# Medical-Image-Analysis-Laboratory/fetalsyngen

Measured on AMD Instinct MI355X. Metric: synthetic volumes/sec at 256^3 (full deform+GMM+blur+resample path), higher is better.
Workload: dtype f32; 1 GPU; BASELINE configs[1]: single 256^3 label volume per step, full path, all gates on; rng=keyed, outputs=fp32 [0,1] image + fp32 labels in HBM, volumes_per_rank=936, parallelism=1 independent replicas (no collective), streams_per_gpu=1

## Files before the change

### fetalsyngen_amd/_build.py

```python
from __future__ import annotations

import os
import shutil
import subprocess
from pathlib import Path

PKG = Path(__file__).resolve().parent
CSRC = PKG / "csrc"
LIB = PKG / "libfsg_hip.so"
SOURCES = ["fsg_deform.hip", "fsg_warp_lean.hip", "fsg_zoom.hip", "fsg_intensity.hip", "fsg_blur.hip", "fsg_blur_rs.hip", "fsg_reduce.hip", "fsg_slice_acq.hip", "fsg_slice_acq_bwd.hip", "fsg_slice_acq_adjoint_bwd.hip", "fsg_artifacts.hip", "fsg_keyed.hip", "fsg_codes.hip", "fsg_seedgen.hip",
           "fsg_regrid.hip", "fsg_pick.hip", "fsg_pipeline.cpp"]
EXTRA = os.environ.get("FSG_EXTRA_FLAGS", "").split()
FLAGS = ["-O3", "--offload-arch=gfx950", "-ffp-contract=off", "-fPIC", "-std=c++17", "-Wall", "-Wno-unused-function"]


def hipcc() -> str:
    exe = shutil.which("hipcc") or "/opt/rocm/bin/hipcc"
    if not os.path.exists(exe):
        raise RuntimeError("hipcc not found: libfsg_hip.so cannot be built")
    return exe


def needs_build() -> bool:
    if not LIB.exists():
        return True
    t = LIB.stat().st_mtime
    deps = [CSRC / s for s in SOURCES] + [CSRC / "fsg_common.h", CSRC / "fsg_sa.h", PKG.parent / "include" / "fsg_hip.h"]
    return any(d.stat().st_mtime > t for d in deps)


def build(force: bool = False, verbose: bool = False) -> Path:
    if not force and not needs_build():
        return LIB
    cc = hipcc()
    objs, jobs = [], []
    build_dir = PKG / "build"
    build_dir.mkdir(exist_ok=True)
    for s in SOURCES:
        o = build_dir / (s + ".o")
        lang = ["-x", "hip"] if s.endswith(".cpp") else []
        cmd = [cc, *FLAGS, *EXTRA, *lang, "-c", str(CSRC / s), "-o", str(o)]
        objs.append(str(o))
        deps = [CSRC / s, CSRC / "fsg_common.h", CSRC / "fsg_sa.h", PKG.parent / "include" / "fsg_hip.h", Path(__file__)]
        if not force and not EXTRA and o.exists() and all(d.stat().st_mtime < o.stat().st_mtime for d in deps):
            continue
        jobs.append(cmd)
    from concurrent.futures import ThreadPoolExecutor

    def run(cmd):
        if verbose:
            print(" ".join(cmd))
        subprocess.run(cmd, check=True)

    with ThreadPoolExecutor(max_workers=min(4, max(len(jobs), 1))) as pool:
        list(pool.map(run, jobs))
    tmp = LIB.with_suffix(".so.tmp")
    subprocess.run([cc, "-shared", "-fPIC", "--offload-arch=gfx950", *objs, "-o", str(tmp)], check=True)
    os.replace(tmp, LIB)
    return LIB


if __name__ == "__main__":
    print(build(force=True, verbose=True))
```

### fetalsyngen_amd/csrc/fsg_deform.hip

```cpp
#include "fsg_common.h"
#include "fsg_ride.h"

int g_tuning_flags = 0;

namespace {

__global__ __launch_bounds__(256) void coords_minmax_kernel(FsgDeformK D, int32_t* __restrict__ mm6) {
  float lo[3] = {INFINITY, INFINITY, INFINITY}, hi[3] = {-INFINITY, -INFINITY, -INFINITY};
  const int rows = D.n0 * D.n1;
  for (int r = blockIdx.x; r < rows; r += gridDim.x) {
    const int i = r / D.n1, j = r - i * D.n1;
    for (int k = threadIdx.x; k < D.n2; k += blockDim.x) {
      float x, y, z;
      fsg_position(D, i, j, k, x, y, z);
      lo[0] = fminf(lo[0], x); hi[0] = fmaxf(hi[0], x);
      lo[1] = fminf(lo[1], y); hi[1] = fmaxf(hi[1], y);
      lo[2] = fminf(lo[2], z); hi[2] = fmaxf(hi[2], z);
    }
  }
  __shared__ float red[6][4];
  const int wave = threadIdx.x >> 6, lane = threadIdx.x & 63;
#pragma unroll
  for (int a = 0; a < 3; ++a) {
    float l = fsg_wave_min(lo[a]), h = fsg_wave_max(hi[a]);
// ... 270 lines not shown
    float v = red[a][0];
    for (int w = 1; w < 4; ++w) v = fminf(v, red[a][w]);
    fsg_atomic_min_key(&mm3[a], v);
  }
}

__global__ __launch_bounds__(256) void coords_faces_min_kernel(FsgDeformK D, int32_t* __restrict__ mm3) {
  __shared__ float red[3][4];
  coords_faces_min_body(D, mm3, red, blockIdx.x, gridDim.x);
}

struct HeadGmm {
  const uint8_t* l0; const uint8_t* l1; const uint8_t* l2; const uint8_t* l3;
  size_t n;
  const float* mus; const float* sigmas; int ntab;
  const float* noise; uint64_t seed, stream_id;
  float* out;
  int ntuples, stride;
  uint32_t sel;
};

__global__ __launch_bounds__(256) __attribute__((amdgpu_waves_per_eu(8, 8))) void sample_head_kernel(HeadGmm G, FsgDeformK D, EpiK E, float* __restrict__ rows,
                                                          int stride, int rows_gx, int nrows, int nfaces,
                                                          int32_t* __restrict__ mm3) {
  __shared__ float s_mu[256], s_sg[256];
  __shared__ float red[3][4];
  union HeadSmem {
    RowsSmem rows;
    float2 code_ms[FSG_CODES_MAX];
  };
  __shared__ HeadSmem U;
  RowsSmem& S = U.rows;
  int b = blockIdx.x;
  if (b < nfaces) {
    coords_faces_min_body(D, mm3, red, b, nfaces);
    return;
  }
  b -= nfaces;
  if (b < nrows) {
    deform_rows_block(D, E, rows, stride, b / rows_gx, (b % rows_gx) * RB_J, S);
    return;
  }
  b -= nrows;
  if (G.ntuples > 0) {
    const fsg_ride::GmmCodesK C{G.l0, G.l1, G.ntuples, G.stride, G.sel, G.n, G.mus, G.sigmas, G.ntab, G.seed, G.stream_id, G.out};
    fsg_ride::gmm_codes_job(C, U.code_ms, (unsigned)b, gridDim.x - (unsigned)(nrows + nfaces));
    return;
  }
  for (int t = threadIdx.x; t < 256; t += blockDim.x) {
    s_mu[t] = t < G.ntab ? G.mus[t] : 0.f;
    s_sg[t] = t < G.ntab ? G.sigmas[t] : 0.f;
  }
  __syncthreads();
  fsg_gmm_x4_loop(G.l0, G.l1, G.l2, G.l3, G.n, s_mu, s_sg, G.noise, G.seed, G.stream_id, G.out, (unsigned)b,
                  gridDim.x - (unsigned)(nrows + nfaces));
}

constexpr int WARP_ROWS_PER_WAVE = 4;

#ifndef FSG_WARP_BATCH
#define FSG_WARP_BATCH 2
#endif
#ifndef FSG_WARP_NO_SKIP_OUTSIDE
#define FSG_WARP_SKIP_OUTSIDE 1
#endif

template <typename LT, bool HAS_LIN, bool HAS_NN, bool FAST, int Q0, int NQ>
__device__ __forceinline__ void warp_emitN(const FsgDeformK& D, const EpiK& E, const Margins& m, const float* sm,
                                           int nf, int i, int j, int kbase, const fsg_tap (&ck)[4],
                                           const fsg_tap (&cbk)[4], size_t row, const float* __restrict__ src_lin,
                                           float* __restrict__ out_lin, const LT* __restrict__ src_nn,
                                           LT* __restrict__ out_nn) {
  const float hx = (float)(D.n0 - 1), hy = (float)(D.n1 - 1), hz = (float)(D.n2 - 1);
  const unsigned sx = (unsigned)D.n1 * (unsigned)D.n2, sy = (unsigned)D.n2;
  float x[NQ], y[NQ], z[NQ];
#pragma unroll
  for (int q = 0; q < NQ; ++q) {
    const int k = min(kbase + 64 * (Q0 + q), D.n2 - 1);
// ... 240 lines not shown
    fsg_tap ck[4] = {none, none, none, none}, cbk[4] = {none, none, none, none};
#pragma unroll
    for (int q = 0; q < PATCH_NQ; ++q) {
      const int k = min(kk + 64 * q, D.n2 - 1);
      ck[q] = tap_at(s_tz, D.tz, D.field != nullptr, k);
      cbk[q] = tap_at(s_bz, E.bz, E.bias != nullptr, k);
    }
    if (live_row)
      warp_emitN<LT, HAS_LIN, HAS_NN, FAST, 0, PATCH_NQ>(D, E, m, sm, nf, i, j, kk, ck, cbk, row, src_lin, out_lin, src_nn,
                                                         out_nn);
    __syncthreads();
  }
}

template <bool MIN_ONLY>
__device__ __forceinline__ void coords_minmax_rows_body(const FsgDeformK& D, int32_t* __restrict__ mm6, int rows_per_block, int blk);

template <bool MIN_ONLY>
__global__ __launch_bounds__(256) void coords_minmax_rows_kernel(FsgDeformK D, int32_t* __restrict__ mm6,
                                                                 int rows_per_block) {
  coords_minmax_rows_body<MIN_ONLY>(D, mm6, rows_per_block, (int)blockIdx.x);
}

__global__ __launch_bounds__(256) void floormin_ride_kernel(FsgDeformK D, int32_t* __restrict__ mm6, int rows_per_block, int nrest,
                                                            const fsg_ride::DrawK P) {
  if ((int)blockIdx.x < nrest) coords_minmax_rows_body<true>(D, mm6, rows_per_block, (int)blockIdx.x);
  else fsg_ride::keyed_draw_body(P, (int)blockIdx.x - nrest);
}

template <bool MIN_ONLY>
__device__ __forceinline__ void coords_minmax_rows_body(const FsgDeformK& D, int32_t* __restrict__ mm6, int rows_per_block, int blk) {
  if (MIN_ONLY) {
    const int32_t one = fsg_f2key(1.0f);
    const int32_t k0 = __hip_atomic_load(&mm6[0], __ATOMIC_RELAXED, __HIP_MEMORY_SCOPE_AGENT);
    const int32_t k1 = __hip_atomic_load(&mm6[1], __ATOMIC_RELAXED, __HIP_MEMORY_SCOPE_AGENT);
    const int32_t k2 = __hip_atomic_load(&mm6[2], __ATOMIC_RELAXED, __HIP_MEMORY_SCOPE_AGENT);
    if (k0 < one && k1 < one && k2 < one) return;
  }
  __shared__ float sm_all[4][ROWCAP];
  __shared__ float red[6][4];
  const int wave = __builtin_amdgcn_readfirstlane(threadIdx.x >> 6), lane = threadIdx.x & 63;
  float* sm = sm_all[wave];
  float lo[3] = {INFINITY, INFINITY, INFINITY}, hi[3] = {-INFINITY, -INFINITY, -INFINITY};
  const int rows = D.n0 * D.n1;
  const int r_begin = blk * rows_per_block;
  const int r_end = min(rows, r_begin + rows_per_block);
  const fsg_tap none = fsg_tap{0, 0, 0.f, 0.f};
  const bool cached = D.n2 <= 256;
  fsg_tap ck[4];
  if (cached) {
#pragma unroll
    for (int q = 0; q < 4; ++q) {
// ... 239 lines not shown
    grid = (rows + rpb - 1) / rpb;
    hipLaunchKernelGGL(coords_minmax_rows_kernel<true>, dim3(grid), dim3(256), 0, st, D, mm3, rpb);
  } else {
    return FSG_E_TOOBIG;
  }
  FSG_RETURN_LAUNCH();
}

int fsg_coords_floormin_rest_f32(const fsg_deform* d, int32_t* mm3, void* stream) {
  FsgDeformK D;
  int rc = fsg_fill_deform(d, D);
  if (rc) return rc;
  if (!mm3) return FSG_E_BADARG;
  if ((D.field ? 3 * D.f2 : 0) > ROWCAP) return FSG_E_TOOBIG;
  const int rows = D.n0 * D.n1;
  int grid = (rows + 7) / 8 < 512 ? (rows + 7) / 8 : 512;
  const int rpb = (rows + grid - 1) / grid;
  grid = (rows + rpb - 1) / rpb;
  hipLaunchKernelGGL(coords_minmax_rows_kernel<true>, dim3(grid), dim3(256), 0, fsg_stream(stream), D, mm3, rpb);
  FSG_RETURN_LAUNCH();
}

static int launch_sample_head(const HeadGmm& G, size_t n, const fsg_deform* d, const fsg_epilogue* epi, float* rows,
                              int row_stride, int32_t* mm3, void* stream);

extern "C" int fsg_internal_floormin_rest_ride(const fsg_deform* d, int32_t* mm3, const void* drawk, unsigned draw_blocks, void* stream) {
  FsgDeformK D;
  int rc = fsg_fill_deform(d, D);
  if (rc) return rc;
  if (!mm3 || !drawk || draw_blocks == 0 || draw_blocks > 4096) return FSG_E_BADARG;
  if ((D.field ? 3 * D.f2 : 0) > ROWCAP) return FSG_E_TOOBIG;
  const int rows = D.n0 * D.n1;
  int grid = (rows + 7) / 8 < 512 ? (rows + 7) / 8 : 512;
  const int rpb = (rows + grid - 1) / grid;
  grid = (rows + rpb - 1) / rpb;
  hipLaunchKernelGGL(floormin_ride_kernel, dim3((unsigned)grid + draw_blocks), dim3(256), 0, fsg_stream(stream), D, mm3, rpb, grid,
                     *reinterpret_cast<const fsg_ride::DrawK*>(drawk));
  FSG_RETURN_LAUNCH();
}

extern "C" int fsg_internal_head_no_gmm(size_t n, const fsg_deform* d, const fsg_epilogue* epi, float* rows, int row_stride,
                                        int32_t* mm3, void* stream) {
  if (n == 0 || !mm3) return FSG_E_BADARG;
  HeadGmm G{};
  G.n = n;
  return launch_sample_head(G, n, d, epi, rows, row_stride, mm3, stream);
}

int fsg_sample_head_f32(const uint8_t* l0, const uint8_t* l1, const uint8_t* l2, const uint8_t* l3, size_t n,
                        const float* mus, const float* sigmas, int ntab, const float* noise, uint64_t seed,
                        uint64_t stream_id, float* out, const fsg_deform* d, const fsg_epilogue* epi, float* rows,
                        int row_stride, int32_t* mm3, void* stream) {
  if (n == 0 || !l0 || !mus || !sigmas || !out || ntab <= 0 || ntab > 256 || !mm3) return FSG_E_BADARG;
  const uintptr_t al = (uintptr_t)l0 | (uintptr_t)l1 | (uintptr_t)l2 | (uintptr_t)l3;
  if ((al & 3) || ((uintptr_t)out & 15)) return FSG_E_ALIGN;
  HeadGmm G{l0, l1, l2, l3, n, mus, sigmas, ntab, noise, seed, stream_id, out, 0, 0, 0u};
  return launch_sample_head(G, n, d, epi, rows, row_stride, mm3, stream);
}

int fsg_sample_head_codes_f32(const uint16_t* codes, const uint8_t* tuples, int ntuples, int stride, const int32_t sel[4],
                              size_t n, const float* mus, const float* sigmas, int ntab, uint64_t seed, uint64_t stream_id,
                              float* out, const fsg_deform* d, const fsg_epilogue* epi, float* rows, int row_stride,
                              int32_t* mm3, void* stream) {
  if (n == 0 || !codes || !tuples || !sel || !mus || !sigmas || !out || ntab <= 0 || ntab > 256 || !mm3) return FSG_E_BADARG;
  if (ntuples <= 0 || stride <= 0 || stride > 256) return FSG_E_BADARG;
  for (int m = 0; m < 4; ++m)
    if (sel[m] < 0 || sel[m] >= stride) return FSG_E_BADARG;
  if (ntuples > FSG_CODES_MAX || n > ((size_t)1 << 30)) return FSG_E_TOOBIG;
  if ((n & 7) || ((uintptr_t)codes & 15) || ((uintptr_t)out & 15)) return FSG_E_ALIGN;
  HeadGmm G{reinterpret_cast<const uint8_t*>(codes), tuples, nullptr, nullptr, n, mus, sigmas, ntab, nullptr, seed, stream_id, out,
            ntuples, stride, (uint32_t)sel[0] | ((uint32_t)sel[1] << 8) | ((uint32_t)sel[2] << 16) | ((uint32_t)sel[3] << 24)};
  return launch_sample_head(G, n, d, epi, rows, row_stride, mm3, stream);
}

static int launch_sample_head(const HeadGmm& G, size_t n, const fsg_deform* d, const fsg_epilogue* epi, float* rows,
                              int row_stride, int32_t* mm3, void* stream) {
  FsgDeformK D;
  int rc = fsg_fill_deform(d, D);
  if (rc) return rc;
  EpiK E;
  rc = fill_epilogue(epi, E);
  if (rc) return rc;
  const int need = (D.field ? 3 * D.f2 : 0) + (E.bias ? E.b2 : 0);
  if (need > 0 && (!rows || row_stride < need)) return FSG_E_BADARG;
  if ((size_t)D.n0 * D.n1 * D.n2 != n) return FSG_E_BADARG;
  if ((D.field ? 3 * D.f2 : 0) > ROWCAP) return FSG_E_TOOBIG;
  if (!rows_block_fits(D, E)) return FSG_E_TOOBIG;
  const int rows_gx = need > 0 ? (D.n1 + RB_J - 1) / RB_J : 0;
  const long long nrows = (long long)rows_gx * D.n0;
  const int faces = faces_total(D.n0, D.n1, D.n2);
  int nfaces = (faces + 255) / 256;
  if (nfaces > 1024) nfaces = 1024;
  size_t ngmm = ((n + 3) / 4 + 255) / 256;
  if (!G.out) ngmm = 0;
  if (ngmm > 4096) ngmm = 4096;
  if (nrows > 1000000) return FSG_E_TOOBIG;
  hipLaunchKernelGGL(sample_head_kernel, dim3((unsigned)(nrows + nfaces + ngmm)), dim3(256), 0, fsg_stream(stream), G, D,
                     E, rows, row_stride, rows_gx > 0 ? rows_gx : 1, (int)nrows, nfaces, mm3);
  FSG_RETURN_LAUNCH();
}

int fsg_coords_f32(const fsg_deform* d, const int32_t* mm6, float* xx, float* yy, float* zz, void* stream) {
  FsgDeformK D;
  int rc = fsg_fill_deform(d, D);
  if (rc) return rc;
  if (!mm6 || !xx || !yy || !zz) return FSG_E_BADARG;
  hipLaunchKernelGGL(coords_kernel, fsg_grid3(D.n0, D.n1, D.n2), fsg_block3(), 0, fsg_stream(stream), D, mm6, xx,
                     yy, zz);
  FSG_RETURN_LAUNCH();
}

int fsg_warp_f32(const fsg_deform* d, const int32_t* mm6, const float* src_lin, float* out_lin,
                 const float* src_nn, float* out_nn, const fsg_epilogue* epi, void* stream) {
  return launch_warp<float>(d, mm6, src_lin, out_lin, src_nn, out_nn, epi, stream);
}

int fsg_warp_f32_u8(const fsg_deform* d, const int32_t* mm6, const float* src_lin, float* out_lin,
                    const uint8_t* src_nn, uint8_t* out_nn, const fsg_epilogue* epi, void* stream) {
  return launch_warp<uint8_t>(d, mm6, src_lin, out_lin, src_nn, out_nn, epi, stream);
}

// ... 57 lines not shown
```

### fetalsyngen_amd/csrc/fsg_keyed.hip

```cpp
#include <hip/hip_runtime.h>
#include <cmath>
#include <cstring>
#include <new>
#include "fsg_common.h"
#include "fsg_ride.h"

namespace {

constexpr int KT_CAP = 1024;

struct KeyedCtx {
  fsg_keyed_config cfg;
  const fsg_tap* tab[4][3][KT_CAP + 1];
  int64_t block_bytes;
  int max_field[3], max_bias[3];
};

struct U4 { uint32_t x, y, z, w; };
inline U4 philox_host(uint32_t c0, uint32_t c1, uint32_t c2, uint32_t c3, uint32_t k0, uint32_t k1) {
  const uint32_t M0 = 0xD2511F53u, M1 = 0xCD9E8D57u, W0 = 0x9E3779B9u, W1 = 0xBB67AE85u;
  for (int r = 0; r < 10; ++r) {
    const uint64_t p0 = (uint64_t)M0 * c0, p1 = (uint64_t)M1 * c2;
    const uint32_t h0 = (uint32_t)(p0 >> 32), l0 = (uint32_t)p0, h1 = (uint32_t)(p1 >> 32), l1 = (uint32_t)p1;
    const uint32_t n0 = h1 ^ c1 ^ k0, n2 = h0 ^ c3 ^ k1;
// ... 161 lines not shown
  }
  if (slot_u(key, S_NOISE_GATE) < c.noise_prob || has(FSG_KO_NOISE_STD)) {
    d.noise_active = 1;
    d.noise_std = has(FSG_KO_NOISE_STD) ? o->noise_std : c.noise_std_min + (c.noise_std_max - c.noise_std_min) * slot_u(key, S_NOISE_STD);
    if (!std::isfinite(d.noise_std)) return FSG_E_BADARG;
    d.noise_std32 = (float)d.noise_std;
  }
  auto align256l = [](int64_t v) { return (v + 255) & ~(int64_t)255; };
  int64_t off = 0;
  d.off_mm8 = (int32_t)off; off = align256l(off + 8 * 4);
  d.off_slots = (int32_t)off; off = align256l(off + FSG_MM_NSLOTS * FSG_MM_SLOT_STRIDE * 4);
  d.off_mus = (int32_t)off; off = align256l(off + 256 * 4);
  d.off_sigmas = (int32_t)off; off = align256l(off + 256 * 4);
  d.off_bias = (int32_t)off; off = align256l(off + (d.bias_active ? (int64_t)d.bias_dims[0] * d.bias_dims[1] * d.bias_dims[2] * 4 : 0));
  if (off > 0x7FFFFF00LL) return FSG_E_TOOBIG;
  d.off_field = (int32_t)off; off = align256l(off + (d.nonlinear ? (int64_t)d.field_dims[0] * d.field_dims[1] * d.field_dims[2] * 12 : 0));
  if (off > 0x7FFFFF00LL) return FSG_E_TOOBIG;
  d.block_bytes = (int32_t)off;
  return 0;
}

using fsg_ride::DrawK;

__global__ __launch_bounds__(256) void keyed_draw_kernel(const DrawK P) { fsg_ride::keyed_draw_body(P, (int)blockIdx.x); }

int fill_draw(const KeyedCtx& C, const fsg_keyed_draws& d, void* block_dev, DrawK& P, unsigned& grid) {
  if (!block_dev || ((uintptr_t)block_dev & 15)) return FSG_E_BADARG;
  char* base = (char*)block_dev;
  P.key = d.key;
  P.mm8 = (int32_t*)(base + d.off_mm8);
  P.slots = (int32_t*)(base + d.off_slots);
  P.mus = (float*)(base + d.off_mus);
  P.sigmas = (float*)(base + d.off_sigmas);
  P.bias = (float*)(base + d.off_bias);
  P.field = (float*)(base + d.off_field);
  P.nlabels = C.cfg.nlabels; P.nseed = C.cfg.n_seed_labels; P.tie = C.cfg.tie_classes;
  P.nbias = d.bias_active ? d.bias_dims[0] * d.bias_dims[1] * d.bias_dims[2] : 0;
  P.nfield = d.nonlinear ? d.field_dims[0] * d.field_dims[1] * d.field_dims[2] * 3 : 0;
  P.bias_std = (float)d.bf_std;
  P.field_std = (float)d.nonlin_std;
  std::memcpy(P.seed_labels, C.cfg.seed_labels, 256);
  std::memcpy(P.gen_classes, C.cfg.generation_classes, 256);
  P.mus_in = (const float*)(uintptr_t)d.mus_in;
  P.sigmas_in = (const float*)(uintptr_t)d.sigmas_in;
  const int work = ((P.nbias + 3) >> 2) + ((P.nfield + 3) >> 2);
  grid = 1u + (unsigned)((work + 255) / 256);
  return 0;
}

int launch_draw(const KeyedCtx& C, const fsg_keyed_draws& d, void* block_dev, void* stream) {
  DrawK P;
  unsigned grid = 0;
  const int rc = fill_draw(C, d, block_dev, P, grid);
  if (rc) return rc;
  hipLaunchKernelGGL(keyed_draw_kernel, dim3(grid), dim3(256), 0, fsg_stream(stream), P);
  FSG_RETURN_LAUNCH();
}

}

extern "C" {

int fsg_keyed_create(const fsg_keyed_config* cfg, void** ctx) {
  if (!cfg || !ctx) return FSG_E_BADARG;
  const fsg_keyed_config& c = *cfg;
  for (int a = 0; a < 3; ++a)
    if (c.shape[a] <= 0 || c.shape[a] > KT_CAP || c.size[a] <= 0 || !(c.resolution[a] > 0)) return FSG_E_BADARG;
  if (c.meta_labels < 1 || c.meta_labels > 4 || c.min_subclusters < 1 || c.max_subclusters < c.min_subclusters ||
      c.max_subclusters - c.min_subclusters >= 16)
    return FSG_E_BADARG;
// ... 34 lines not shown
  KeyedCtx* K = (KeyedCtx*)ctx;
  if (!K || kind < 0 || kind > 3 || axis < 0 || axis > 2 || n < 1 || n > KT_CAP) return FSG_E_BADARG;
  K->tab[kind][axis][n] = table_dev;
  return 0;
}

int64_t fsg_keyed_block_bytes(void* ctx) { return ctx ? ((KeyedCtx*)ctx)->block_bytes : (int64_t)FSG_E_BADARG; }

int fsg_keyed_draw(void* ctx, uint64_t key, fsg_keyed_draws* out) {
  if (!ctx || !out) return FSG_E_BADARG;
  return draw(*(KeyedCtx*)ctx, key, nullptr, *out);
}

int fsg_keyed_draw_with(void* ctx, uint64_t key, const fsg_keyed_overrides* overrides, fsg_keyed_draws* out) {
  if (!ctx || !out) return FSG_E_BADARG;
  return draw(*(KeyedCtx*)ctx, key, overrides, *out);
}

int fsg_keyed_fill_block(void* ctx, const fsg_keyed_draws* d, void* block_dev, void* stream) {
  if (!ctx || !d) return FSG_E_BADARG;
  return launch_draw(*(KeyedCtx*)ctx, *d, block_dev, stream);
}

int fsg_keyed_sample_run(void* ctx, const int64_t* iv, int niv, fsg_keyed_draws* draws_out, void* stream) {
  KeyedCtx* K = (KeyedCtx*)ctx;
  if (!K || !iv || niv < FSG_KEYED_I_COUNT) return FSG_E_BADARG;
  const fsg_keyed_config& c = K->cfg;
  fsg_keyed_draws d;
  const bool ext = niv >= FSG_KEYED_I_COUNT_OV;
  const fsg_keyed_overrides* ov = ext ? (const fsg_keyed_overrides*)(uintptr_t)iv[FSG_KEYED_I_OVERRIDES] : nullptr;
  int rc = draw(*K, (uint64_t)iv[FSG_KEYED_I_KEY], ov, d);
  if (rc) return rc;
  if (draws_out) *draws_out = d;
  const int64_t cap = ext && iv[FSG_KEYED_I_BLOCK_BYTES] > 0 ? iv[FSG_KEYED_I_BLOCK_BYTES] : K->block_bytes;
  if (d.block_bytes > cap) return FSG_E_TOOBIG;
  char* base = (char*)(uintptr_t)iv[FSG_KEYED_I_BLOCK];
  if (!base) return FSG_E_BADARG;

  fsg_sample_plan q;
  std::memset(&q, 0, sizeof q);
  for (int a = 0; a < 3; ++a) q.shape[a] = c.shape[a];
  fsg_sample_image im;
  im.prior_in = (const float*)(uintptr_t)iv[FSG_KEYED_I_PRIOR_IN];
  im.image_in = (const float*)(uintptr_t)iv[FSG_KEYED_I_IMAGE_IN];
  im.image_out = (float*)(uintptr_t)iv[FSG_KEYED_I_IMAGE_OUT];
  if (im.image_in && !im.image_out) return FSG_E_BADARG;
// ... 84 lines not shown
  q.mm8_preset = 1;
  q.mm_slots = d.resample_active ? (int32_t*)(base + d.off_slots) : nullptr;
  q.mm_nslots = d.resample_active ? FSG_MM_NSLOTS : 0;
  q.out = (float*)(uintptr_t)iv[FSG_KEYED_I_OUT];
  q.trace_events = (void**)(uintptr_t)iv[FSG_KEYED_I_TRACE_EVENTS];
  q.trace_ids = (int32_t*)(uintptr_t)iv[FSG_KEYED_I_TRACE_IDS];
  q.trace_cap = (int32_t)iv[FSG_KEYED_I_TRACE_CAP];
  q.ev_blur_begin = (void*)(uintptr_t)iv[FSG_KEYED_I_EV_BLUR_BEGIN];
  q.ev_blur_end = (void*)(uintptr_t)iv[FSG_KEYED_I_EV_BLUR_END];

  const int64_t flags = iv[FSG_KEYED_I_FLAGS];
  const bool draw_done = (flags & 1) != 0 && !ov;
  DrawK next_draw;
  int32_t rode = 0;
  char* nbase = (char*)(uintptr_t)iv[FSG_KEYED_I_NEXT_BLOCK];
  if (nbase && (flags & 4)) {
    fsg_keyed_draws dn;
    rc = draw(*K, (uint64_t)iv[FSG_KEYED_I_NEXT_KEY], nullptr, dn);
    if (rc) return rc;
    if (dn.block_bytes > K->block_bytes) return FSG_E_TOOBIG;
    unsigned grid = 0;
    rc = fill_draw(*K, dn, nbase, next_draw, grid);
    if (rc) return rc;
    q.ride_draw = &next_draw;
    q.ride_draw_blocks = grid;
    q.rode = &rode;
  }

  if (!draw_done && q.trace_events && q.trace_ids && q.trace_cap > 1) {
    hipError_t e = hipEventRecord((hipEvent_t)q.trace_events[0], fsg_stream(stream));
    if (e != hipSuccess) return (int)e;
    q.trace_ids[0] = FSG_ST_BEGIN;
    q.trace_ids[q.trace_cap] = 1;
    q.trace_start = 1;
    q.trace_first_id = FSG_ST_DRAW;
  }
  if (!draw_done) {
    rc = launch_draw(*K, d, base, stream);
    if (rc) return rc;
  }
  rc = fsg_sample_run_image(&q, &im, stream);
  if (draws_out) draws_out->rode = rode;
  return rc;
}

}
```

### fetalsyngen_amd/csrc/fsg_pipeline.cpp

```cpp
#include <hip/hip_runtime.h>
#include <cstddef>
#include "../../include/fsg_hip.h"

extern "C" int fsg_internal_floormin_rest_ride(const fsg_deform* d, int32_t* mm3, const void* drawk, unsigned draw_blocks, void* stream);
extern "C" int fsg_internal_head_no_gmm(size_t n, const fsg_deform* d, const fsg_epilogue* epi, float* rows, int row_stride,
                                        int32_t* mm3, void* stream);


extern int g_tuning_flags;

extern "C" int fsg_pipeline_teardown(void) { return 0; }

#define FSG_TRY(expr)        \
  do {                       \
    int rc_ = (expr);        \
    if (rc_ != 0) return rc_; \
  } while (0)
#define FSG_HIP(expr)                          \
  do {                                         \
    hipError_t e_ = (expr);                    \
    if (e_ != hipSuccess) return (int)e_;      \
  } while (0)

extern "C" int fsg_sample_run(const fsg_sample_plan* p, void* stream) { return fsg_sample_run_image(p, nullptr, stream); }

extern "C" int fsg_sample_run_image(const fsg_sample_plan* p, const fsg_sample_image* im, void* stream) {
  if (!p || !p->out || !p->ws0 || !p->ws1 || !p->mm8) return FSG_E_BADARG;
  const int n0 = p->shape[0], n1 = p->shape[1], n2 = p->shape[2];
  if (n0 <= 0 || n1 <= 0 || n2 <= 0) return FSG_E_BADARG;
  const size_t n = (size_t)n0 * n1 * n2;
  if (n > (size_t)0x7FFFFFFF) return FSG_E_TOOBIG;
  const float* const image_in = im ? im->image_in : nullptr;
  float* const image_out = im ? im->image_out : nullptr;
  if (image_in && !image_out) return FSG_E_BADARG;
  const float* const prior = im ? im->prior_in : nullptr;
  hipStream_t st = (hipStream_t)stream;
  int rode = 0;
  if (p->rode) *p->rode = 0;

  int ntrace = p->trace_start > 0 ? p->trace_start : 0;
  auto mark = [&](int id) -> int {
    if (!p->trace_events || !p->trace_ids || ntrace >= p->trace_cap) return 0;
    hipError_t e = hipEventRecord((hipEvent_t)p->trace_events[ntrace], st);
    if (e != hipSuccess) return (int)e;
    p->trace_ids[ntrace++] = id;
    p->trace_ids[p->trace_cap] = ntrace;
    return 0;
  };
  FSG_TRY(mark(p->trace_start > 0 ? p->trace_first_id : FSG_ST_BEGIN));

  const bool has_gamma = p->epi.gamma > 0.f, has_bias = p->epi.bias != nullptr;
  bool head_done = false;
  fsg_deform dh = p->deform;
  const int need_h = 3 * dh.field_dims[2] + (has_bias ? p->epi.bias_dims[2] : 0);
  const bool fused_head = p->deform_active && p->mm8_preset && p->ws_rows && !(g_tuning_flags & FSG_TUNE_SPLIT_HEAD) &&
                          need_h > 0 && need_h <= p->row_stride;
  if (p->arena_host) {
    if (!p->arena_dev || (p->arena_bytes & 15)) return FSG_E_BADARG;
    FSG_TRY(fsg_copy_bytes(p->arena_dev, p->arena_host, (size_t)p->arena_bytes, stream));
    FSG_TRY(mark(FSG_ST_UPLOAD));
  }
  int head_rc = 0;
  if (fused_head) {
    dh.rows = nullptr;
    dh.row_stride = 0;
    head_rc = FSG_E_ALIGN;
    if (prior)
      head_rc = fsg_internal_head_no_gmm(n, &dh, &p->epi, p->ws_rows, p->row_stride, p->mm8, stream);
    else if (p->label_codes && p->code_tuples && !p->gmm_noise && !(g_tuning_flags & FSG_TUNE_NO_SEED_CODES))
      head_rc = fsg_sample_head_codes_f32(p->label_codes, p->code_tuples, p->code_ntuples, p->code_stride, p->code_sel, n, p->mus,
                                          p->sigmas, p->ntab, p->gmm_seed, p->gmm_stream, p->ws0, &dh, &p->epi, p->ws_rows,
                                          p->row_stride, p->mm8, stream);
    if (!prior && (head_rc == FSG_E_ALIGN || head_rc == FSG_E_TOOBIG))
      head_rc = fsg_sample_head_f32(p->label_parts[0], p->label_parts[1], p->label_parts[2], p->label_parts[3], n, p->mus,
                                    p->sigmas, p->ntab, p->gmm_noise, p->gmm_seed, p->gmm_stream, p->ws0, &dh, &p->epi,
                                    p->ws_rows, p->row_stride, p->mm8, stream);
    if (head_rc == 0) head_done = true;
    if (head_done) FSG_TRY(mark(FSG_ST_HEAD));
  }
  if (head_rc != 0 && head_rc != FSG_E_TOOBIG && head_rc != FSG_E_ALIGN) return head_rc;
  if (!head_done && prior) {
    if (!p->mm8_preset) FSG_TRY(fsg_minmax_init(p->mm8, 4, 4, stream));
  } else if (!head_done)
    FSG_TRY(fsg_gmm_sample_u8x4_mm(p->label_parts[0], p->label_parts[1], p->label_parts[2], p->label_parts[3], n,
                                   p->mus, p->sigmas, p->ntab, p->gmm_noise, p->gmm_seed, p->gmm_stream, p->ws0,
                                   p->mm8_preset ? nullptr : p->mm8, 4, 4, stream));
  if (!head_done && !prior) FSG_TRY(mark(FSG_ST_GMM));
  float* cur = prior ? const_cast<float*>(prior) : p->ws0;
  float* other = prior ? p->ws0 : p->ws1;
  auto rotate = [&]() {
    float* t = cur;
    cur = other;
    other = t == prior ? p->ws1 : t;
  };

  if (p->deform_active) {
    if (!p->seg_in || (!p->seg_out && !p->seg_out_u8) || (p->seg_out_u8 && !p->seg_in_u8)) return FSG_E_BADARG;
    fsg_deform d = p->deform;
    const int need = 3 * d.field_dims[2] + (has_bias ? p->epi.bias_dims[2] : 0);
    if (head_done) {
      d.rows = p->ws_rows;
      d.row_stride = p->row_stride;
      if (p->ride_draw && p->ride_draw_blocks) {
        FSG_TRY(fsg_internal_floormin_rest_ride(&d, p->mm8, p->ride_draw, p->ride_draw_blocks, stream));
        rode |= 1;
      } else {
        FSG_TRY(fsg_coords_floormin_rest_f32(&d, p->mm8, stream));
      }
      FSG_TRY(mark(FSG_ST_FLOORMIN));
    } else {
      if (p->ws_rows && need > 0 && need <= p->row_stride) {
        d.rows = nullptr;
        d.row_stride = 0;
        FSG_TRY(fsg_deform_rows_f32(&d, &p->epi, p->ws_rows, p->row_stride, stream));
        FSG_TRY(mark(FSG_ST_ROWS));
        d.rows = p->ws_rows;
        d.row_stride = p->row_stride;
      } else {
        d.rows = nullptr;
        d.row_stride = 0;
      }
      int rc = fsg_coords_floormin_f32(&d, p->mm8, stream);
      if (rc == FSG_E_TOOBIG) {
        return FSG_E_TOOBIG;
      }
      FSG_TRY(rc);
      FSG_TRY(mark(FSG_ST_FLOORMIN));
    }
    int rw = FSG_E_ALIGN;
    bool image_done = false;
    if (image_in) {
      if (p->seg_out_u8)
// ... 240 lines not shown
```

### fetalsyngen_amd/csrc/fsg_ride.h

```cpp
#pragma once
#include "fsg_common.h"

#define FSG_MM_NSLOTS 64

namespace fsg_ride {

constexpr int32_t KEY_POS_INF = 0x7F800000, KEY_NEG_INF = (int32_t)0x807FFFFF;

struct DrawK {
  uint64_t key;
  int32_t* mm8;
  int32_t* slots;
  float* mus;
  float* sigmas;
  float* bias;
  float* field;
  int nlabels, nseed, tie, nbias, nfield;
  float bias_std, field_std;
  uint8_t seed_labels[256];
  uint8_t gen_classes[256];
  const float* mus_in;
  const float* sigmas_in;
};

__device__ __forceinline__ float keyed_uniform(uint64_t key, uint64_t stream, uint32_t e) {
  const uint32_t blk = e >> 2;
  const uint4 r = fsg_philox4x32_10(blk, 0u, (uint32_t)stream, (uint32_t)(stream >> 32), (uint32_t)key, (uint32_t)(key >> 32));
  const uint32_t w = (e & 3) == 0 ? r.x : ((e & 3) == 1 ? r.y : ((e & 3) == 2 ? r.z : r.w));
  return (float)(w >> 8) * 5.9604644775390625e-08f;
}

__device__ __forceinline__ void keyed_draw_body(const DrawK& P, const int blk) {
  const int tid = threadIdx.x;
  if (blk == 0) {
    if (tid < 8) P.mm8[tid] = tid < 4 ? KEY_POS_INF : KEY_NEG_INF;
    for (int q = tid; q < FSG_MM_NSLOTS * FSG_MM_SLOT_STRIDE; q += 256) {
      const int f = q % FSG_MM_SLOT_STRIDE;
      P.slots[q] = f == 0 ? KEY_POS_INF : (f == 1 ? KEY_NEG_INF : 0);
    }
    __shared__ float s_mu[256];
    float sg = 0.f;
    if (tid < P.nlabels) {
      s_mu[tid] = P.mus_in ? P.mus_in[tid] : 25.f + 200.f * keyed_uniform(P.key, 5, (uint32_t)tid);
      sg = P.sigmas_in ? P.sigmas_in[tid] : 5.f + 20.f * keyed_uniform(P.key, 5, (uint32_t)(P.nlabels + tid));
    }
    __syncthreads();
    float tied = 0.f;
    if (P.tie && tid < P.nseed) {
      tied = s_mu[P.gen_classes[tid]] + 25.f * fsg_randn1(P.key, 6, (uint64_t)tid);
      tied = fminf(fmaxf(tied, 0.f), 225.f);
    }
    __syncthreads();
    if (P.tie && tid < P.nseed) s_mu[P.seed_labels[tid]] = tied;
    __syncthreads();
    if (tid < P.nlabels) {
      P.mus[tid] = s_mu[tid];
      P.sigmas[tid] = sg;
    }
    return;
  }
  const int t = (blk - 1) * 256 + tid;
  const int nb4 = (P.nbias + 3) >> 2, nf4 = (P.nfield + 3) >> 2;
  if (t < nb4) {
// ... 54 lines not shown
```

### include/fsg_hip.h

```cpp
#ifndef FSG_HIP_H
#define FSG_HIP_H

#include <stddef.h>
#include <stdint.h>

#ifdef __cplusplus
extern "C" {
#endif

#define FSG_ABI_VERSION 8

#define FSG_E_BADARG (-1)
#define FSG_E_TOOBIG (-2)
#define FSG_E_ALIGN  (-3)
#define FSG_E_NOTABLE (-4)

typedef struct fsg_tap {
  int32_t lo;
  int32_t hi;
  float w_lo;
  float w_hi;
} fsg_tap;

struct fsg_epilogue;
// ... 12 lines not shown
  const float* rows;
  int32_t row_stride;
} fsg_deform;

int fsg_abi_version(void);
const char* fsg_error_string(int code);

#define FSG_TUNE_GENERIC_WARP 1
#define FSG_TUNE_PRECISE_MATH 2
#define FSG_TUNE_GENERIC_ZOOM 4
#define FSG_TUNE_NO_PREFETCH 8
#define FSG_TUNE_NO_PATCH 32
#define FSG_TUNE_ROW_ZOOM 256
#define FSG_TUNE_TILE_ZOOM 512
#define FSG_TUNE_NO_BLUR_FUSE 1024
#define FSG_TUNE_SA_DIRECT 128
#define FSG_TUNE_SPLIT_HEAD 2048
#define FSG_TUNE_SLAB_ZOOM 8192
#define FSG_TUNE_NO_LEAN 4096
#define FSG_TUNE_NO_SEED_CODES 65536
#define FSG_TUNE_SA_FWD_DIRECT 131072
#define FSG_TUNE_SA_FWD_PLATE 262144
#define FSG_TUNE_NO_BLUR_RS 16384
int fsg_set_tuning(int flags);
int fsg_warp_set_variant(int variant);

int fsg_randn_f32(float* out, size_t n, uint64_t seed, uint64_t stream_id, void* stream);

int fsg_gmm_sample_u8(const uint8_t* labels, size_t n, const float* mus, const float* sigmas, int ntab,
                      const float* noise, uint64_t seed, uint64_t stream_id, float* out, void* stream);
int fsg_gmm_sample_i64(const int64_t* labels, size_t n, const float* mus, const float* sigmas, int ntab,
                       const float* noise, uint64_t seed, uint64_t stream_id, float* out, void* stream);
int fsg_gmm_sample_u8x4(const uint8_t* l0, const uint8_t* l1, const uint8_t* l2, const uint8_t* l3, size_t n,
                        const float* mus, const float* sigmas, int ntab, const float* noise, uint64_t seed,
                        uint64_t stream_id, float* out, void* stream);
int fsg_gmm_sample_u8x4_mm(const uint8_t* l0, const uint8_t* l1, const uint8_t* l2, const uint8_t* l3, size_t n,
                           const float* mus, const float* sigmas, int ntab, const float* noise, uint64_t seed,
                           uint64_t stream_id, float* out, int32_t* mm, int nmin, int nmax, void* stream);

int fsg_label_stats_u8(const uint8_t* labels, const float* values, size_t n, int nlabels,
                       unsigned long long* count, double* sum, double* sumsq, void* stream);

int fsg_zoom3d_f32(const float* src, int sx, int sy, int sz, int nch, const fsg_tap* tx, const fsg_tap* ty,
                   const fsg_tap* tz, float* dst, int dx, int dy, int dz, void* stream);

int fsg_resample_noise_f32(const float* src, int sx, int sy, int sz, const fsg_tap* tx, const fsg_tap* ty,
// ... 402 lines not shown
```

Baseline: 4614 volumes/s.

## Fold next-step keyed draw into head kernel and skip settled floor-min pass

Moves the next volume's keyed draw blocks out of the separate floor-min ride kernel and into the fused head kernel's grid. Adds a host-side bound check that recomputes the corner field values from the Philox key. When the check proves the lower bound is already settled, the floor-min-rest kernel launch is skipped entirely. This removes one kernel launch and a coordinate pass per step, at the cost of host work per key and a correctness dependence on the conservative bound.

```diff
diff --git a/fetalsyngen_amd/_build.py b/fetalsyngen_amd/_build.py
--- a/fetalsyngen_amd/_build.py
+++ b/fetalsyngen_amd/_build.py
@@ -25,7 +25,7 @@
     if not LIB.exists():
         return True
     t = LIB.stat().st_mtime
-    deps = [CSRC / s for s in SOURCES] + [CSRC / "fsg_common.h", CSRC / "fsg_sa.h", PKG.parent / "include" / "fsg_hip.h"]
+    deps = [CSRC / s for s in SOURCES] + [CSRC / "fsg_common.h", CSRC / "fsg_ride.h", CSRC / "fsg_sa.h", PKG.parent / "include" / "fsg_hip.h"]
     return any(d.stat().st_mtime > t for d in deps)
 
 
@@ -41,7 +41,7 @@
         lang = ["-x", "hip"] if s.endswith(".cpp") else []
         cmd = [cc, *FLAGS, *EXTRA, *lang, "-c", str(CSRC / s), "-o", str(o)]
         objs.append(str(o))
-        deps = [CSRC / s, CSRC / "fsg_common.h", CSRC / "fsg_sa.h", PKG.parent / "include" / "fsg_hip.h", Path(__file__)]
+        deps = [CSRC / s, CSRC / "fsg_common.h", CSRC / "fsg_ride.h", CSRC / "fsg_sa.h", PKG.parent / "include" / "fsg_hip.h", Path(__file__)]
         if not force and not EXTRA and o.exists() and all(d.stat().st_mtime < o.stat().st_mtime for d in deps):
             continue
         jobs.append(cmd)
diff --git a/fetalsyngen_amd/csrc/fsg_deform.hip b/fetalsyngen_amd/csrc/fsg_deform.hip
--- a/fetalsyngen_amd/csrc/fsg_deform.hip
+++ b/fetalsyngen_amd/csrc/fsg_deform.hip
@@ -316,7 +316,7 @@
 
 __global__ __launch_bounds__(256) __attribute__((amdgpu_waves_per_eu(8, 8))) void sample_head_kernel(HeadGmm G, FsgDeformK D, EpiK E, float* __restrict__ rows,
                                                           int stride, int rows_gx, int nrows, int nfaces,
-                                                          int32_t* __restrict__ mm3) {
+                                                          int32_t* __restrict__ mm3, int ndraw, const fsg_ride::DrawK P) {
   __shared__ float s_mu[256], s_sg[256];
   __shared__ float red[3][4];
   union HeadSmem {
@@ -331,6 +331,11 @@
     return;
   }
   b -= nfaces;
+  if (b < ndraw) {
+    fsg_ride::keyed_draw_body(P, b, s_mu);
+    return;
+  }
+  b -= ndraw;
   if (b < nrows) {
     deform_rows_block(D, E, rows, stride, b / rows_gx, (b % rows_gx) * RB_J, S);
     return;
@@ -338,7 +343,7 @@
   b -= nrows;
   if (G.ntuples > 0) {
     const fsg_ride::GmmCodesK C{G.l0, G.l1, G.ntuples, G.stride, G.sel, G.n, G.mus, G.sigmas, G.ntab, G.seed, G.stream_id, G.out};
-    fsg_ride::gmm_codes_job(C, U.code_ms, (unsigned)b, gridDim.x - (unsigned)(nrows + nfaces));
+    fsg_ride::gmm_codes_job(C, U.code_ms, (unsigned)b, gridDim.x - (unsigned)(nrows + nfaces + ndraw));
     return;
   }
   for (int t = threadIdx.x; t < 256; t += blockDim.x) {
@@ -347,7 +352,7 @@
   }
   __syncthreads();
   fsg_gmm_x4_loop(G.l0, G.l1, G.l2, G.l3, G.n, s_mu, s_sg, G.noise, G.seed, G.stream_id, G.out, (unsigned)b,
-                  gridDim.x - (unsigned)(nrows + nfaces));
+                  gridDim.x - (unsigned)(nrows + nfaces + ndraw));
 }
 
 constexpr int WARP_ROWS_PER_WAVE = 4;
@@ -634,12 +639,6 @@
   coords_minmax_rows_body<MIN_ONLY>(D, mm6, rows_per_block, (int)blockIdx.x);
 }
 
-__global__ __launch_bounds__(256) void floormin_ride_kernel(FsgDeformK D, int32_t* __restrict__ mm6, int rows_per_block, int nrest,
-                                                            const fsg_ride::DrawK P) {
-  if ((int)blockIdx.x < nrest) coords_minmax_rows_body<true>(D, mm6, rows_per_block, (int)blockIdx.x);
-  else fsg_ride::keyed_draw_body(P, (int)blockIdx.x - nrest);
-}
-
 template <bool MIN_ONLY>
 __device__ __forceinline__ void coords_minmax_rows_body(const FsgDeformK& D, int32_t* __restrict__ mm6, int rows_per_block, int blk) {
   if (MIN_ONLY) {
@@ -925,46 +924,32 @@
 }
 
 static int launch_sample_head(const HeadGmm& G, size_t n, const fsg_deform* d, const fsg_epilogue* epi, float* rows,
-                              int row_stride, int32_t* mm3, void* stream);
-
-extern "C" int fsg_internal_floormin_rest_ride(const fsg_deform* d, int32_t* mm3, const void* drawk, unsigned draw_blocks, void* stream) {
-  FsgDeformK D;
-  int rc = fsg_fill_deform(d, D);
-  if (rc) return rc;
-  if (!mm3 || !drawk || draw_blocks == 0 || draw_blocks > 4096) return FSG_E_BADARG;
-  if ((D.field ? 3 * D.f2 : 0) > ROWCAP) return FSG_E_TOOBIG;
-  const int rows = D.n0 * D.n1;
-  int grid = (rows + 7) / 8 < 512 ? (rows + 7) / 8 : 512;
-  const int rpb = (rows + grid - 1) / grid;
-  grid = (rows + rpb - 1) / rpb;
-  hipLaunchKernelGGL(floormin_ride_kernel, dim3((unsigned)grid + draw_blocks), dim3(256), 0, fsg_stream(stream), D, mm3, rpb, grid,
-                     *reinterpret_cast<const fsg_ride::DrawK*>(drawk));
-  FSG_RETURN_LAUNCH();
-}
+                              int row_stride, int32_t* mm3, const void* drawk, unsigned draw_blocks, void* stream);
 
 extern "C" int fsg_internal_head_no_gmm(size_t n, const fsg_deform* d, const fsg_epilogue* epi, float* rows, int row_stride,
-                                        int32_t* mm3, void* stream) {
+                                        int32_t* mm3, const void* drawk, unsigned draw_blocks, void* stream) {
   if (n == 0 || !mm3) return FSG_E_BADARG;
   HeadGmm G{};
   G.n = n;
-  return launch_sample_head(G, n, d, epi, rows, row_stride, mm3, stream);
-}
-
-int fsg_sample_head_f32(const uint8_t* l0, const uint8_t* l1, const uint8_t* l2, const uint8_t* l3, size_t n,
-                        const float* mus, const float* sigmas, int ntab, const float* noise, uint64_t seed,
-                        uint64_t stream_id, float* out, const fsg_deform* d, const fsg_epilogue* epi, float* rows,
-                        int row_stride, int32_t* mm3, void* stream) {
+  return launch_sample_head(G, n, d, epi, rows, row_stride, mm3, drawk, draw_blocks, stream);
+}
+
+extern "C" int fsg_internal_head_f32(const uint8_t* l0, const uint8_t* l1, const uint8_t* l2, const uint8_t* l3, size_t n,
+                                     const float* mus, const float* sigmas, int ntab, const float* noise, uint64_t seed,
+                                     uint64_t stream_id, float* out, const fsg_deform* d, const fsg_epilogue* epi, float* rows,
+                                     int row_stride, int32_t* mm3, const void* drawk, unsigned draw_blocks, void* stream) {
   if (n == 0 || !l0 || !mus || !sigmas || !out || ntab <= 0 || ntab > 256 || !mm3) return FSG_E_BADARG;
   const uintptr_t al = (uintptr_t)l0 | (uintptr_t)l1 | (uintptr_t)l2 | (uintptr_t)l3;
   if ((al & 3) || ((uintptr_t)out & 15)) return FSG_E_ALIGN;
   HeadGmm G{l0, l1, l2, l3, n, mus, sigmas, ntab, noise, seed, stream_id, out, 0, 0, 0u};
-  return launch_sample_head(G, n, d, epi, rows, row_stride, mm3, stream);
-}
-
-int fsg_sample_head_codes_f32(const uint16_t* codes, const uint8_t* tuples, int ntuples, int stride, const int32_t sel[4],
-                              size_t n, const float* mus, const float* sigmas, int ntab, uint64_t seed, uint64_t stream_id,
-                              float* out, const fsg_deform* d, const fsg_epilogue* epi, float* rows, int row_stride,
-                              int32_t* mm3, void* stream) {
+  return launch_sample_head(G, n, d, epi, rows, row_stride, mm3, drawk, draw_blocks, stream);
+}
+
+extern "C" int fsg_internal_head_codes_f32(const uint16_t* codes, const uint8_t* tuples, int ntuples, int stride,
+                                           const int32_t sel[4], size_t n, const float* mus, const float* sigmas, int ntab,
+                                           uint64_t seed, uint64_t stream_id, float* out, const fsg_deform* d,
+                                           const fsg_epilogue* epi, float* rows, int row_stride, int32_t* mm3, const void* drawk,
+                                           unsigned draw_blocks, void* stream) {
   if (n == 0 || !codes || !tuples || !sel || !mus || !sigmas || !out || ntab <= 0 || ntab > 256 || !mm3) return FSG_E_BADARG;
   if (ntuples <= 0 || stride <= 0 || stride > 256) return FSG_E_BADARG;
   for (int m = 0; m < 4; ++m)
@@ -973,17 +958,34 @@
   if ((n & 7) || ((uintptr_t)codes & 15) || ((uintptr_t)out & 15)) return FSG_E_ALIGN;
   HeadGmm G{reinterpret_cast<const uint8_t*>(codes), tuples, nullptr, nullptr, n, mus, sigmas, ntab, nullptr, seed, stream_id, out,
             ntuples, stride, (uint32_t)sel[0] | ((uint32_t)sel[1] << 8) | ((uint32_t)sel[2] << 16) | ((uint32_t)sel[3] << 24)};
-  return launch_sample_head(G, n, d, epi, rows, row_stride, mm3, stream);
+  return launch_sample_head(G, n, d, epi, rows, row_stride, mm3, drawk, draw_blocks, stream);
+}
+
+int fsg_sample_head_f32(const uint8_t* l0, const uint8_t* l1, const uint8_t* l2, const uint8_t* l3, size_t n,
+                        const float* mus, const float* sigmas, int ntab, const float* noise, uint64_t seed,
+                        uint64_t stream_id, float* out, const fsg_deform* d, const fsg_epilogue* epi, float* rows,
+                        int row_stride, int32_t* mm3, void* stream) {
+  return fsg_internal_head_f32(l0, l1, l2, l3, n, mus, sigmas, ntab, noise, seed, stream_id, out, d, epi, rows, row_stride, mm3,
+                               nullptr, 0u, stream);
+}
+
+int fsg_sample_head_codes_f32(const uint16_t* codes, const uint8_t* tuples, int ntuples, int stride, const int32_t sel[4],
+                              size_t n, const float* mus, const float* sigmas, int ntab, uint64_t seed, uint64_t stream_id,
+                              float* out, const fsg_deform* d, const fsg_epilogue* epi, float* rows, int row_stride,
+                              int32_t* mm3, void* stream) {
+  return fsg_internal_head_codes_f32(codes, tuples, ntuples, stride, sel, n, mus, sigmas, ntab, seed, stream_id, out, d, epi, rows,
+                                     row_stride, mm3, nullptr, 0u, stream);
 }
 
 static int launch_sample_head(const HeadGmm& G, size_t n, const fsg_deform* d, const fsg_epilogue* epi, float* rows,
-                              int row_stride, int32_t* mm3, void* stream) {
+                              int row_stride, int32_t* mm3, const void* drawk, unsigned draw_blocks, void* stream) {
   FsgDeformK D;
   int rc = fsg_fill_deform(d, D);
   if (rc) return rc;
   EpiK E;
   rc = fill_epilogue(epi, E);
   if (rc) return rc;
+  if (drawk ? (draw_blocks == 0 || draw_blocks > FSG_HEAD_DRAW_MAX) : draw_blocks != 0) return FSG_E_BADARG;
   const int need = (D.field ? 3 * D.f2 : 0) + (E.bias ? E.b2 : 0);
   if (need > 0 && (!rows || row_stride < need)) return FSG_E_BADARG;
   if ((size_t)D.n0 * D.n1 * D.n2 != n) return FSG_E_BADARG;
@@ -998,8 +1000,10 @@
   if (!G.out) ngmm = 0;
   if (ngmm > 4096) ngmm = 4096;
   if (nrows > 1000000) return FSG_E_TOOBIG;
-  hipLaunchKernelGGL(sample_head_kernel, dim3((unsigned)(nrows + nfaces + ngmm)), dim3(256), 0, fsg_stream(stream), G, D,
-                     E, rows, row_stride, rows_gx > 0 ? rows_gx : 1, (int)nrows, nfaces, mm3);
+  static const fsg_ride::DrawK no_draw = {};
+  hipLaunchKernelGGL(sample_head_kernel, dim3((unsigned)(nrows + nfaces + ngmm) + draw_blocks), dim3(256), 0, fsg_stream(stream), G,
+                     D, E, rows, row_stride, rows_gx > 0 ? rows_gx : 1, (int)nrows, nfaces, mm3, (int)draw_blocks,
+                     drawk ? *reinterpret_cast<const fsg_ride::DrawK*>(drawk) : no_draw);
   FSG_RETURN_LAUNCH();
 }
 
diff --git a/fetalsyngen_amd/csrc/fsg_keyed.hip b/fetalsyngen_amd/csrc/fsg_keyed.hip
--- a/fetalsyngen_amd/csrc/fsg_keyed.hip
+++ b/fetalsyngen_amd/csrc/fsg_keyed.hip
@@ -207,7 +207,10 @@
 
 using fsg_ride::DrawK;
 
-__global__ __launch_bounds__(256) void keyed_draw_kernel(const DrawK P) { fsg_ride::keyed_draw_body(P, (int)blockIdx.x); }
+__global__ __launch_bounds__(256) void keyed_draw_kernel(const DrawK P) {
+  __shared__ float s_mu[256];
+  fsg_ride::keyed_draw_body(P, (int)blockIdx.x, s_mu);
+}
 
 int fill_draw(const KeyedCtx& C, const fsg_keyed_draws& d, void* block_dev, DrawK& P, unsigned& grid) {
   if (!block_dev || ((uintptr_t)block_dev & 15)) return FSG_E_BADARG;
@@ -231,6 +234,74 @@
   const int work = ((P.nbias + 3) >> 2) + ((P.nfield + 3) >> 2);
   grid = 1u + (unsigned)((work + 255) / 256);
   return 0;
+}
+
+double field_value_host(uint64_t key, float field_std, uint32_t e) {
+  const U4 r = philox_host(e >> 2, 0u, 3u, 0u, (uint32_t)key, (uint32_t)(key >> 32));
+  const double S = 5.9604644775390625e-08;
+  const bool second = (e & 2u) != 0;
+  const double u = (double)(((second ? r.z : r.x) >> 8) + 1u) * S, t = (double)((second ? r.w : r.y) >> 8) * S;
+  const double rad = std::sqrt(-2.0 * std::log(u)), ang = 6.283185307179586476925286766559 * t;
+  return (double)field_std * (rad * ((e & 1u) ? std::sin(ang) : std::cos(ang)));
+}
+
+bool floormin_settled(const fsg_keyed_config& c, const fsg_keyed_draws& d) {
+  if (!d.deform_active) return false;
+  const bool field = d.nonlinear && d.field_dims[0] > 0 && d.field_dims[1] > 0 && d.field_dims[2] > 0;
+  if (d.nonlinear && !field) return false;
+  if (field)
+    for (int a = 0; a < 3; ++a)
+      if (d.field_dims[a] > c.shape[a]) return false;
+  const float field_std = (float)d.nonlin_std;
+  bool settled[3] = {false, false, false};
+  for (int corner = 0; corner < 8 && !(settled[0] && settled[1] && settled[2]); ++corner) {
+    double p[3], lo[3] = {0, 0, 0}, hi[3] = {0, 0, 0};
+    int node0[3], nodes[3];
+    for (int a = 0; a < 3; ++a) {
+      const bool last = (corner >> a) & 1;
+      p[a] = (double)(last ? c.shape[a] - 1 : 0) - (double)(float)((c.size[a] - 1) / 2.0);
+      const int f = field ? d.field_dims[a] : 1;
+      nodes[a] = f < 2 ? f : 2;
+      node0[a] = last ? f - nodes[a] : 0;
+    }
+    if (field) {
+      bool useful = false;
+      for (int a = 0; a < 3; ++a) {
+        const float* A = d.A + 3 * a;
+        const double x = (double)A[0] * p[0] + (double)A[1] * p[1] + (double)A[2] * p[2] + (double)(float)d.c2[a];
+        if (!settled[a] && x < 1.0) useful = true;
+      }
+      if (!useful) continue;
+      for (int ch = 0; ch < 3; ++ch) {
+        lo[ch] = INFINITY;
+        hi[ch] = -INFINITY;
+      }
+      for (int i = 0; i < nodes[0]; ++i)
+        for (int j = 0; j < nodes[1]; ++j)
+          for (int k = 0; k < nodes[2]; ++k) {
+            const uint32_t node = (uint32_t)(((node0[0] + i) * d.field_dims[1] + node0[1] + j) * d.field_dims[2] + node0[2] + k);
+            for (uint32_t ch = 0; ch < 3; ++ch) {
+              const double v = field_value_host(d.key, field_std, 3u * node + ch);
+              lo[ch] = std::fmin(lo[ch], v);
+              hi[ch] = std::fmax(hi[ch], v);
+              if (!(v == v)) lo[ch] = hi[ch] = NAN;
+            }
+          }
+    }
+    for (int a = 0; a < 3; ++a) {
+      if (settled[a]) continue;
+      const float* A = d.A + 3 * a;
+      double ub = (double)(float)d.c2[a], mag = std::fabs(ub);
+      for (int ch = 0; ch < 3; ++ch) {
+        const double w = (double)A[ch], t0 = w * (p[ch] + lo[ch]), t1 = w * (p[ch] + hi[ch]);
+        ub += std::fmax(t0, t1);
+        mag += std::fmax(std::fabs(t0), std::fabs(t1));
+        if (!(t0 == t0) || !(t1 == t1)) ub = NAN;
+      }
+      if (ub < 1.0 - (0.25 + 1e-4 * mag)) settled[a] = true;
+    }
+  }
+  return settled[0] && settled[1] && settled[2];
 }
 
 int launch_draw(const KeyedCtx& C, const fsg_keyed_draws& d, void* block_dev, void* stream) {
@@ -311,6 +382,17 @@
   return launch_draw(*(KeyedCtx*)ctx, *d, block_dev, stream);
 }
 
+int fsg_internal_sample_run(const fsg_sample_plan* p, const fsg_sample_image* im, int floormin_settled, void* stream);
+
+int fsg_internal_keyed_floormin_settled(void* ctx, uint64_t key, const fsg_keyed_overrides* overrides) {
+  if (!ctx) return FSG_E_BADARG;
+  const KeyedCtx& K = *(KeyedCtx*)ctx;
+  fsg_keyed_draws d;
+  const int rc = draw(K, key, overrides, d);
+  if (rc) return rc < 0 ? rc : -rc;
+  return floormin_settled(K.cfg, d) ? 1 : 0;
+}
+
 int fsg_keyed_sample_run(void* ctx, const int64_t* iv, int niv, fsg_keyed_draws* draws_out, void* stream) {
   KeyedCtx* K = (KeyedCtx*)ctx;
   if (!K || !iv || niv < FSG_KEYED_I_COUNT) return FSG_E_BADARG;
@@ -441,9 +523,11 @@
     unsigned grid = 0;
     rc = fill_draw(*K, dn, nbase, next_draw, grid);
     if (rc) return rc;
-    q.ride_draw = &next_draw;
-    q.ride_draw_blocks = grid;
-    q.rode = &rode;
+    if (grid <= FSG_HEAD_DRAW_MAX) {
+      q.ride_draw = &next_draw;
+      q.ride_draw_blocks = grid;
+      q.rode = &rode;
+    }
   }
 
   if (!draw_done && q.trace_events && q.trace_ids && q.trace_cap > 1) {
@@ -458,7 +542,7 @@
     rc = launch_draw(*K, d, base, stream);
     if (rc) return rc;
   }
-  rc = fsg_sample_run_image(&q, &im, stream);
+  rc = fsg_internal_sample_run(&q, &im, floormin_settled(c, d) ? 1 : 0, stream);
   if (draws_out) draws_out->rode = rode;
   return rc;
 }
diff --git a/fetalsyngen_amd/csrc/fsg_pipeline.cpp b/fetalsyngen_amd/csrc/fsg_pipeline.cpp
--- a/fetalsyngen_amd/csrc/fsg_pipeline.cpp
+++ b/fetalsyngen_amd/csrc/fsg_pipeline.cpp
@@ -2,9 +2,17 @@
 #include <cstddef>
 #include "../../include/fsg_hip.h"
 
-extern "C" int fsg_internal_floormin_rest_ride(const fsg_deform* d, int32_t* mm3, const void* drawk, unsigned draw_blocks, void* stream);
 extern "C" int fsg_internal_head_no_gmm(size_t n, const fsg_deform* d, const fsg_epilogue* epi, float* rows, int row_stride,
-                                        int32_t* mm3, void* stream);
+                                        int32_t* mm3, const void* drawk, unsigned draw_blocks, void* stream);
+extern "C" int fsg_internal_head_f32(const uint8_t* l0, const uint8_t* l1, const uint8_t* l2, const uint8_t* l3, size_t n,
+                                     const float* mus, const float* sigmas, int ntab, const float* noise, uint64_t seed,
+                                     uint64_t stream_id, float* out, const fsg_deform* d, const fsg_epilogue* epi, float* rows,
+                                     int row_stride, int32_t* mm3, const void* drawk, unsigned draw_blocks, void* stream);
+extern "C" int fsg_internal_head_codes_f32(const uint16_t* codes, const uint8_t* tuples, int ntuples, int stride,
+                                           const int32_t sel[4], size_t n, const float* mus, const float* sigmas, int ntab,
+                                           uint64_t seed, uint64_t stream_id, float* out, const fsg_deform* d,
+                                           const fsg_epilogue* epi, float* rows, int row_stride, int32_t* mm3, const void* drawk,
+                                           unsigned draw_blocks, void* stream);
 
 
 extern int g_tuning_flags;
@@ -24,7 +32,12 @@
 
 extern "C" int fsg_sample_run(const fsg_sample_plan* p, void* stream) { return fsg_sample_run_image(p, nullptr, stream); }
 
+extern "C" int fsg_internal_sample_run(const fsg_sample_plan* p, const fsg_sample_image* im, int floormin_settled, void* stream);
 extern "C" int fsg_sample_run_image(const fsg_sample_plan* p, const fsg_sample_image* im, void* stream) {
+  return fsg_internal_sample_run(p, im, 0, stream);
+}
+
+extern "C" int fsg_internal_sample_run(const fsg_sample_plan* p, const fsg_sample_image* im, int floormin_settled, void* stream) {
   if (!p || !p->out || !p->ws0 || !p->ws1 || !p->mm8) return FSG_E_BADARG;
   const int n0 = p->shape[0], n1 = p->shape[1], n2 = p->shape[2];
   if (n0 <= 0 || n1 <= 0 || n2 <= 0) return FSG_E_BADARG;
@@ -61,21 +74,24 @@
     FSG_TRY(mark(FSG_ST_UPLOAD));
   }
   int head_rc = 0;
+  const void* const ride = p->ride_draw && p->ride_draw_blocks ? p->ride_draw : nullptr;
+  const unsigned ride_blocks = ride ? p->ride_draw_blocks : 0u;
   if (fused_head) {
     dh.rows = nullptr;
     dh.row_stride = 0;
     head_rc = FSG_E_ALIGN;
     if (prior)
-      head_rc = fsg_internal_head_no_gmm(n, &dh, &p->epi, p->ws_rows, p->row_stride, p->mm8, stream);
+      head_rc = fsg_internal_head_no_gmm(n, &dh, &p->epi, p->ws_rows, p->row_stride, p->mm8, ride, ride_blocks, stream);
     else if (p->label_codes && p->code_tuples && !p->gmm_noise && !(g_tuning_flags & FSG_TUNE_NO_SEED_CODES))
-      head_rc = fsg_sample_head_codes_f32(p->label_codes, p->code_tuples, p->code_ntuples, p->code_stride, p->code_sel, n, p->mus,
-                                          p->sigmas, p->ntab, p->gmm_seed, p->gmm_stream, p->ws0, &dh, &p->epi, p->ws_rows,
-                                          p->row_stride, p->mm8, stream);
+      head_rc = fsg_internal_head_codes_f32(p->label_codes, p->code_tuples, p->code_ntuples, p->code_stride, p->code_sel, n, p->mus,
+                                            p->sigmas, p->ntab, p->gmm_seed, p->gmm_stream, p->ws0, &dh, &p->epi, p->ws_rows,
+                                            p->row_stride, p->mm8, ride, ride_blocks, stream);
     if (!prior && (head_rc == FSG_E_ALIGN || head_rc == FSG_E_TOOBIG))
-      head_rc = fsg_sample_head_f32(p->label_parts[0], p->label_parts[1], p->label_parts[2], p->label_parts[3], n, p->mus,
-                                    p->sigmas, p->ntab, p->gmm_noise, p->gmm_seed, p->gmm_stream, p->ws0, &dh, &p->epi,
-                                    p->ws_rows, p->row_stride, p->mm8, stream);
+      head_rc = fsg_internal_head_f32(p->label_parts[0], p->label_parts[1], p->label_parts[2], p->label_parts[3], n, p->mus,
+                                      p->sigmas, p->ntab, p->gmm_noise, p->gmm_seed, p->gmm_stream, p->ws0, &dh, &p->epi,
+                                      p->ws_rows, p->row_stride, p->mm8, ride, ride_blocks, stream);
     if (head_rc == 0) head_done = true;
+    if (head_done && ride) rode |= 1;
     if (head_done) FSG_TRY(mark(FSG_ST_HEAD));
   }
   if (head_rc != 0 && head_rc != FSG_E_TOOBIG && head_rc != FSG_E_ALIGN) return head_rc;
@@ -101,13 +117,10 @@
     if (head_done) {
       d.rows = p->ws_rows;
       d.row_stride = p->row_stride;
-      if (p->ride_draw && p->ride_draw_blocks) {
-        FSG_TRY(fsg_internal_floormin_rest_ride(&d, p->mm8, p->ride_draw, p->ride_draw_blocks, stream));
-        rode |= 1;
-      } else {
+      if (!floormin_settled || (g_tuning_flags & FSG_TUNE_NO_FLOORMIN_SKIP)) {
         FSG_TRY(fsg_coords_floormin_rest_f32(&d, p->mm8, stream));
+        FSG_TRY(mark(FSG_ST_FLOORMIN));
       }
-      FSG_TRY(mark(FSG_ST_FLOORMIN));
     } else {
       if (p->ws_rows && need > 0 && need <= p->row_stride) {
         d.rows = nullptr;
diff --git a/fetalsyngen_amd/csrc/fsg_ride.h b/fetalsyngen_amd/csrc/fsg_ride.h
--- a/fetalsyngen_amd/csrc/fsg_ride.h
+++ b/fetalsyngen_amd/csrc/fsg_ride.h
@@ -2,6 +2,8 @@
 #include "fsg_common.h"
 
 #define FSG_MM_NSLOTS 64
+
+#define FSG_HEAD_DRAW_MAX 4096u
 
 namespace fsg_ride {
 
@@ -30,7 +32,7 @@
   return (float)(w >> 8) * 5.9604644775390625e-08f;
 }
 
-__device__ __forceinline__ void keyed_draw_body(const DrawK& P, const int blk) {
+__device__ __forceinline__ void keyed_draw_body(const DrawK& P, const int blk, float* s_mu) {
   const int tid = threadIdx.x;
   if (blk == 0) {
     if (tid < 8) P.mm8[tid] = tid < 4 ? KEY_POS_INF : KEY_NEG_INF;
@@ -38,7 +40,6 @@
       const int f = q % FSG_MM_SLOT_STRIDE;
       P.slots[q] = f == 0 ? KEY_POS_INF : (f == 1 ? KEY_NEG_INF : 0);
     }
-    __shared__ float s_mu[256];
     float sg = 0.f;
     if (tid < P.nlabels) {
       s_mu[tid] = P.mus_in ? P.mus_in[tid] : 25.f + 200.f * keyed_uniform(P.key, 5, (uint32_t)tid);
diff --git a/include/fsg_hip.h b/include/fsg_hip.h
--- a/include/fsg_hip.h
+++ b/include/fsg_hip.h
@@ -58,6 +58,7 @@
 #define FSG_TUNE_SA_FWD_DIRECT 131072
 #define FSG_TUNE_SA_FWD_PLATE 262144
 #define FSG_TUNE_NO_BLUR_RS 16384
+#define FSG_TUNE_NO_FLOORMIN_SKIP 524288
 int fsg_set_tuning(int flags);
 int fsg_warp_set_variant(int variant);
 
```

After: 4699 volumes/s, median of 6. 1.02x the previous value.
